# MoFHeka/MeepoEmbedding

Measured on AMD Instinct MI355X. Metric: key-lookups/sec, higher is better.
Workload: dtype int64 keys / fp32 rows (copy)

## Files before the change

include/meepo_embedding.h:

```cpp
#ifndef MEEPO_EMBEDDING_H
#define MEEPO_EMBEDDING_H
#include <stddef.h>
#include <stdint.h>

#ifdef __cplusplus
extern "C" {
#endif

#define MEE_ABI_VERSION 2

#define MEE_EMPTY_KEY     INT64_MIN
#define MEE_RECLAIMED_KEY (INT64_MIN + 1)
#define MEE_BUCKET_WIDTH  16

enum { MEE_OK = 0, MEE_ERR_INVALID_ARG = -1, MEE_ERR_OUT_OF_MEMORY = -2, MEE_ERR_HIP = -3,
       MEE_ERR_NO_DEVICE = -4, MEE_ERR_BATCH_TOO_LARGE = -5, MEE_ERR_UNSUPPORTED = -6,
       MEE_ERR_RCCL = -7  };

enum { MEE_OPT_NONE = 0, MEE_OPT_ADAGRAD = 1, MEE_OPT_ADAM = 2 };
enum { MEE_INIT_CONSTANT = 0, MEE_INIT_UNIFORM = 1 };
enum { MEE_STATUS_TABLE_FULL = 1u, MEE_STATUS_RESERVED_KEY = 2u, MEE_STATUS_STALE_HANDLE = 4u, MEE_STATUS_INTERNAL = 8u };
enum { MEE_MEM_HBM = 0, MEE_MEM_HOST_PINNED = 1 };
enum { MEE_FLAG_TRACK_HITS = 1u, MEE_FLAG_ADMISSION = 2u };

// ... 40 lines not shown
    uint32_t from_env;
    uint32_t placement_consistent;
    float    odd_over_even[2];
    float    block_us_by_index_mod_8[8];
    uint32_t xcc_of_index_mod_8[8];
} mee_calibration;
int mee_device_calibration(int32_t device, mee_calibration* out);

int mee_find(const mee_table* t, const int64_t* d_keys, size_t n, float* d_out, uint8_t* d_found, void* stream);
enum { MEE_FIND_DEFAULT = 0u, MEE_FIND_STREAM_STORES = 1u, MEE_FIND_CACHED_STORES = 2u, MEE_FIND_STREAM_ROWS = 4u, MEE_FIND_STREAM_BUCKETS = 8u };
int mee_find_ex(const mee_table* t, const int64_t* d_keys, size_t n, float* d_out, uint8_t* d_found, uint32_t flags, void* stream);
int mee_find_unordered(const mee_table* t, const int64_t* d_keys, size_t n, float* d_out, uint8_t* d_found, void* stream);
typedef struct mee_find_request { const int64_t* d_keys; size_t n; float* d_out; uint8_t* d_found; } mee_find_request;
int mee_find_many(const mee_table* t, const mee_find_request* reqs, uint32_t count, void* stream);
int mee_find_located(const mee_table* t, const int64_t* d_keys, size_t n, float* d_out, uint8_t* d_found, int64_t* d_slots_out, void* stream);
int mee_find_located_prepare(mee_table* t, const int64_t* d_keys, size_t n, float* d_out, uint8_t* d_found, int64_t* d_slots_out, void* stream);
int mee_find_or_insert_located_prepare(mee_table* t, const int64_t* d_keys, size_t n, float* d_out, uint8_t* d_found, int64_t* d_slots_out, void* stream);
int mee_find_missing(const mee_table* t, const int64_t* d_keys, size_t n, float* d_out, uint8_t* d_found, void* stream);
int mee_find_counted(const mee_table* t, const int64_t* d_keys, size_t n, float* d_out, uint8_t* d_found, int missing_only,
                     void* stream);
int mee_hits_scan(mee_table* t, uint32_t min_hits, uint32_t max_hits, int reset, int64_t* d_keys_out, size_t cap, size_t* n_out,
                  void* stream);
enum { MEE_POOL_SUM = 0, MEE_POOL_MEAN = 1 };
int mee_find_pooled(const mee_table* t, const int64_t* d_keys, size_t n, const uint64_t* d_bag_offsets, size_t n_bags, float* d_out,
                    uint8_t* d_found, int mode, void* stream);
int mee_find_pooled_weighted(const mee_table* t, const int64_t* d_keys, size_t n, const uint64_t* d_bag_offsets, size_t n_bags,
                             const float* d_weights, float* d_out, uint8_t* d_found, int64_t* d_located_out, void* stream);
int mee_pooled_weighted_backward(const mee_table* t, const int64_t* d_keys, const int64_t* d_located, size_t n, const uint64_t* d_bag_offsets,
                                 size_t n_bags, const float* d_weights, const float* d_bag_grads, float* d_grads_out, float* d_weight_grads_out,
                                 void* stream);
enum { MEE_TIER_COUNT_COLD = 1, MEE_TIER_COUNT_HOT = 2 };
int mee_find_pooled_tiered(const mee_table* hot, const mee_table* cold, const int64_t* d_keys, size_t n, const uint64_t* d_bag_offsets, size_t n_bags,
                           void* d_out, uint32_t out_dtype, uint8_t* d_found , int mode, uint32_t flags, void* stream);
int mee_insert(mee_table* t, const int64_t* d_keys, const float* d_values, size_t n, void* stream);
int mee_assign(mee_table* t, const int64_t* d_keys, const float* d_values, size_t n, uint8_t* d_found, void* stream);
int mee_find_plane(const mee_table* t, uint32_t plane, const int64_t* d_keys, size_t n, float* d_out, uint8_t* d_found,
                   void* stream);
int mee_assign_plane(mee_table* t, uint32_t plane, const int64_t* d_keys, const float* d_values, size_t n, uint8_t* d_found,
                     void* stream);
int mee_remove(mee_table* t, const int64_t* d_keys, size_t n, uint8_t* d_found, void* stream);
int mee_find_or_insert(mee_table* t, const int64_t* d_keys, size_t n, float* d_out, uint8_t* d_found, void* stream);
int mee_find_or_insert_located(mee_table* t, const int64_t* d_keys, size_t n, float* d_out, uint8_t* d_found, int64_t* d_slots_out, void* stream);
int mee_find_or_insert_admit(mee_table* t, const int64_t* d_keys, size_t n, float* d_out, uint8_t* d_found, uint32_t min_count, void* stream);
int mee_admission_decay(mee_table* t, uint32_t shift, void* stream);
int mee_insert_missing(mee_table* t, const int64_t* d_keys, const float* d_values, size_t n, const uint8_t* d_found, void* stream);
int mee_find_or_insert_missing(mee_table* t, const int64_t* d_keys, size_t n, float* d_out, const uint8_t* d_found, void* stream);
int mee_export(const mee_table* t, int64_t* d_keys_out, float* d_values_out, float* d_state1_out,
               float* d_state2_out, size_t cap, size_t* n_out, void* stream);
int mee_export_range(const mee_table* t, uint64_t slot_begin, uint64_t slot_end, int64_t* d_keys_out, float* d_values_out,
                     float* d_state1_out, float* d_state2_out, size_t cap, size_t* n_out, void* stream);
int mee_reserve(mee_table* t, uint64_t new_capacity, void* stream);
int mee_size(const mee_table* t, size_t* n_out, void* stream);
int mee_status(const mee_table* t, uint32_t* bits_out, void* stream);
int mee_clear_status(mee_table* t, void* stream);
int mee_locate(const mee_table* t, const int64_t* d_keys, size_t n, int64_t* d_slots_out, uint8_t* d_found, void* stream);
int mee_table_plane(const mee_table* t, uint32_t plane, void** ptr_out, uint64_t* row_stride_bytes, uint32_t* value_memory);
int mee_probe_length(const mee_table* t, const int64_t* d_keys, size_t n, uint64_t* buckets_visited_out, void* stream);
int mee_probe_histogram(const mee_table* t, const int64_t* d_keys, size_t n, uint64_t* hist_out , void* stream);

typedef struct mee_group mee_group;
int mee_group_create(mee_table* const* tables, uint32_t n_tables, uint64_t max_apply_batch, mee_group** out);
int mee_group_destroy(mee_group* g);
int mee_group_set_tuning(mee_group* g, const char* name, int value);
int mee_find_grouped(mee_group* g, const int64_t* d_keys, const uint64_t* d_offsets, size_t n, float* d_out, uint8_t* d_found,
                     void* stream);
int mee_group_find_or_insert(mee_group* g, const int64_t* d_keys, const uint64_t* d_offsets, size_t n, float* d_out, uint8_t* d_found,
// ... 165 lines not shown
```

meepoembedding_amd/_lib.py:

```python
from __future__ import annotations

import ctypes as C
import os

import torch

_HERE = os.path.dirname(os.path.abspath(__file__))
LIB_PATH = os.environ.get("MEE_LIB_PATH") or os.path.join(_HERE, "libmeepo_hip.so")

OK = 0
ERR_INVALID_ARG, ERR_OUT_OF_MEMORY, ERR_HIP, ERR_NO_DEVICE, ERR_BATCH_TOO_LARGE, ERR_UNSUPPORTED, ERR_RCCL = -1, -2, -3, -4, -5, -6, -7
OPT_NONE, OPT_ADAGRAD, OPT_ADAM = 0, 1, 2
INIT_CONSTANT, INIT_UNIFORM = 0, 1
STATUS_TABLE_FULL, STATUS_RESERVED_KEY, STATUS_STALE_HANDLE, STATUS_INTERNAL = 1, 2, 4, 8
FIND_DEFAULT, FIND_STREAM_STORES, FIND_CACHED_STORES, FIND_STREAM_ROWS, FIND_STREAM_BUCKETS = 0, 1, 2, 4, 8
HANDLE_SLOT_MASK = (1 << 40) - 1
MEM_HBM, MEM_HOST_PINNED = 0, 1
DTYPE_F32, DTYPE_BF16 = 0, 1
FLAG_TRACK_HITS, FLAG_ADMISSION = 1, 2
TIER_COUNT_COLD, TIER_COUNT_HOT = 1, 2
ABI_VERSION = 2
EMPTY_KEY = -(1 << 63)
RECLAIMED_KEY = EMPTY_KEY + 1
BUCKET_WIDTH = 16
# ... 65 lines not shown
    "mee_hits_scan": (C.c_int, [_vp, _u32, _u32, C.c_int, _vp, _sz, C.POINTER(_sz), _vp]),
    "mee_insert": (C.c_int, [_vp, _vp, _vp, _sz, _vp]),
    "mee_insert_missing": (C.c_int, [_vp, _vp, _vp, _sz, _vp, _vp]),
    "mee_find_or_insert_missing": (C.c_int, [_vp, _vp, _sz, _vp, _vp, _vp]),
    "mee_assign": (C.c_int, [_vp, _vp, _vp, _sz, _vp, _vp]),
    "mee_find_plane": (C.c_int, [_vp, _u32, _vp, _sz, _vp, _vp, _vp]),
    "mee_assign_plane": (C.c_int, [_vp, _u32, _vp, _vp, _sz, _vp, _vp]),
    "mee_remove": (C.c_int, [_vp, _vp, _sz, _vp, _vp]),
    "mee_find_or_insert": (C.c_int, [_vp, _vp, _sz, _vp, _vp, _vp]),
    "mee_export": (C.c_int, [_vp, _vp, _vp, _vp, _vp, _sz, C.POINTER(_sz), _vp]),
    "mee_group_create": (C.c_int, [C.POINTER(_vp), _u32, _u64, C.POINTER(_vp)]),
    "mee_group_find_pooled": (C.c_int, [_vp, _vp, _sz, _vp, _sz, _vp, _vp, _vp, C.c_int, _vp]),
    "mee_group_apply_adagrad_pooled": (C.c_int, [_vp, _vp, _vp, _sz, _vp, _vp, _vp, _sz, _f32, _f32, _vp]),
    "mee_group_apply_adam_pooled": (C.c_int, [_vp, _vp, _vp, _sz, _vp, _vp, _vp, _sz, _f32, _f32, _f32, _f32, _u64, _vp]),
    "mee_group_find_pooled_jagged": (C.c_int, [_vp, _vp, _sz, _vp, _sz, _vp, _vp, _vp, _vp, C.c_int, _vp]),
    "mee_group_apply_adagrad_indexed": (C.c_int, [_vp, _vp, _vp, _vp, _sz, _vp, _sz, _f32, _f32, _vp]),
    "mee_group_apply_adam_indexed": (C.c_int, [_vp, _vp, _vp, _vp, _sz, _vp, _sz, _f32, _f32, _f32, _f32, _u64, _vp]),
    "mee_group_find_or_insert": (C.c_int, [_vp, _vp, _vp, _sz, _vp, _vp, _vp]),
    "mee_group_apply_adagrad": (C.c_int, [_vp, _vp, _vp, _vp, _sz, _f32, _f32, _vp]),
    "mee_group_apply_adam": (C.c_int, [_vp, _vp, _vp, _vp, _sz, _f32, _f32, _f32, _f32, _u64, _vp]),
    "mee_group_destroy": (C.c_int, [_vp]),
    "mee_group_set_tuning": (C.c_int, [_vp, C.c_char_p, C.c_int]),
    "mee_find_grouped": (C.c_int, [_vp, _vp, _vp, _sz, _vp, _vp, _vp]),
    "mee_mixed_group_create": (C.c_int, [C.POINTER(_vp), _u32, _u64, C.POINTER(_vp)]),
    "mee_mixed_group_destroy": (C.c_int, [_vp]),
    "mee_mixed_group_layout": (C.c_int, [_vp, _u64, C.POINTER(_u64), C.POINTER(_u64)]),
    "mee_mixed_group_find_pooled": (C.c_int, [_vp, _vp, _sz, _vp, _sz, _vp, _u32, _vp, _vp, C.c_int, C.c_int, _vp]),
    "mee_mixed_group_apply_adagrad_pooled": (C.c_int, [_vp, _vp, _vp, _sz, _vp, _vp, _vp, _sz, _f32, _f32, _vp]),
    "mee_mixed_group_apply_adam_pooled": (C.c_int, [_vp, _vp, _vp, _sz, _vp, _vp, _vp, _sz, _f32, _f32, _f32, _f32, _u64, _vp]),
    "mee_mixed_group_set_tuning": (C.c_int, [_vp, C.c_char_p, C.c_int]),
    "mee_find_pooled": (C.c_int, [_vp, _vp, _sz, _vp, _sz, _vp, _vp, C.c_int, _vp]),
    "mee_find_pooled_weighted": (C.c_int, [_vp, _vp, _sz, _vp, _sz, _vp, _vp, _vp, _vp, _vp]),
    "mee_find_pooled_tiered": (C.c_int, [_vp, _vp, _vp, _sz, _vp, _sz, _vp, _u32, _vp, C.c_int, _u32, _vp]),
    "mee_pooled_weighted_backward": (C.c_int, [_vp, _vp, _vp, _sz, _vp, _sz, _vp, _vp, _vp, _vp, _vp]),
    "mee_group_find_pooled_weighted": (C.c_int, [_vp, _vp, _sz, _vp, _sz, _vp, _vp, _vp, _vp, _vp]),
    "mee_group_pooled_weighted_backward": (C.c_int, [_vp, _vp, _vp, _sz, _vp, _sz, _vp, _vp, _vp, _vp, _vp]),
    "mee_apply_adagrad_indexed": (C.c_int, [_vp, _vp, _vp, _sz, _vp, _sz, _f32, _f32, _vp]),
    "mee_apply_adam_indexed": (C.c_int, [_vp, _vp, _vp, _sz, _vp, _sz, _f32, _f32, _f32, _f32, _u64, _vp]),
    "mee_dedup_keys": (C.c_int, [_vp, _vp, _sz, _vp, _vp, C.c_int64, _vp]),
    "mee_reserve": (C.c_int, [_vp, _u64, _vp]),
    "mee_export_range": (C.c_int, [_vp, _u64, _u64, _vp, _vp, _vp, _vp, _sz, C.POINTER(_sz), _vp]),
    "mee_size": (C.c_int, [_vp, C.POINTER(_sz), _vp]),
    "mee_status": (C.c_int, [_vp, C.POINTER(_u32), _vp]),
    "mee_clear_status": (C.c_int, [_vp, _vp]),
    "mee_find_unordered": (C.c_int, [_vp, _vp, _sz, _vp, _vp, _vp]),
    "mee_find_many": (C.c_int, [_vp, C.POINTER(FindRequest), _u32, _vp]),
    "mee_find_located": (C.c_int, [_vp, _vp, _sz, _vp, _vp, _vp, _vp]),
    "mee_find_or_insert_located": (C.c_int, [_vp, _vp, _sz, _vp, _vp, _vp, _vp]),
    "mee_find_located_prepare": (C.c_int, [_vp, _vp, _sz, _vp, _vp, _vp, _vp]),
    "mee_find_or_insert_located_prepare": (C.c_int, [_vp, _vp, _sz, _vp, _vp, _vp, _vp]),
    "mee_apply_adagrad_located": (C.c_int, [_vp, _vp, _vp, _vp, _sz, _f32, _f32, _vp]),
    "mee_apply_adam_located": (C.c_int, [_vp, _vp, _vp, _vp, _sz, _f32, _f32, _f32, _f32, _u64, _vp]),
    "mee_find_or_insert_admit": (C.c_int, [_vp, _vp, _sz, _vp, _vp, _u32, _vp]),
    "mee_admission_decay": (C.c_int, [_vp, _u32, _vp]),
    "mee_locate": (C.c_int, [_vp, _vp, _sz, _vp, _vp, _vp]),
    "mee_table_plane": (C.c_int, [_vp, _u32, C.POINTER(_vp), C.POINTER(_u64), C.POINTER(_u32)]),
    "mee_device_calibration": (C.c_int, [C.c_int32, C.POINTER(Calibration)]),
    "mee_probe_length": (C.c_int, [_vp, _vp, _sz, C.POINTER(_u64), _vp]),
    "mee_probe_histogram": (C.c_int, [_vp, _vp, _sz, C.POINTER(C.c_uint64), _vp]),
    "mee_apply_adagrad": (C.c_int, [_vp, _vp, _vp, _sz, _f32, _f32, _vp]),
    "mee_apply_adam": (C.c_int, [_vp, _vp, _vp, _sz, _f32, _f32, _f32, _f32, _u64, _vp]),
    "mee_apply_prepare": (C.c_int, [_vp, _vp, _sz, _vp]),
    "mee_apply_discard": (C.c_int, [_vp, _vp]),
    "mee_dedup_sum": (C.c_int, [_vp, _vp, _vp, _sz, _vp, _vp, _vp, _vp, C.c_int64, _vp]),
    "mee_hash_batch": (C.c_int, [_vp, _sz, _u64, _u32, _vp, _vp, _vp, _vp]),
    "mee_router_create": (C.c_int, [_i32, _u64, _u32, C.POINTER(_vp)]),
# ... 80 lines not shown
```

meepoembedding_amd/csrc/meepo_find.hip:

```cpp
#include <hip/hip_runtime.h>
#include <hip/hip_ext.h>

#include <cmath>
#include <cstdlib>
#include <cstring>

#include "meepo_apply_part.h"


namespace mee {


template <int DIM4, int R, int NT>
__device__ __forceinline__ void find_span(const int64_t* __restrict__ tkeys, const f32x4* __restrict__ values, uint64_t nb,
                                          const int64_t* __restrict__ keys, uint64_t n, f32x4* __restrict__ out,
                                          uint8_t* __restrict__ found, float defv, uint32_t dim4_rt, uint32_t* hits,
                                          int64_t* __restrict__ slots_out, uint64_t wave, uint64_t n_waves, int64_t handle_tag = 0) {
    const int lane = threadIdx.x & 63, tile = lane >> 4, tl = lane & 15;
    const uint32_t dim4 = DIM4 ? DIM4 : dim4_rt;
    constexpr int KPW = 4 * R;
    const f32x4 def4 = {defv, defv, defv, defv};

    for (uint64_t base = wave * KPW; base < n; base += n_waves * KPW) {
        int64_t key[R];
// ... 148 lines not shown
                           (uint64_t)(m.first_block[q + 1] - m.first_block[q]) * (blockDim.x >> 6));
}

template <int FLAGS>
__global__ __launch_bounds__(256) void find_missing_kernel(const int64_t* __restrict__ tkeys, const float4* __restrict__ values,
                                                           uint64_t nb, uint32_t dim4, const int64_t* __restrict__ keys, uint64_t n,
                                                           float4* __restrict__ out, uint8_t* __restrict__ found, uint32_t* hits) {
    const int lane = threadIdx.x & 63, tile = lane >> 4, tl = lane & 15;
    const uint64_t wave = (uint64_t)blockIdx.x * (blockDim.x >> 6) + (threadIdx.x >> 6);
    const uint64_t n_waves = (uint64_t)gridDim.x * (blockDim.x >> 6);
    for (uint64_t base = wave * 64; base < n; base += n_waves * 64) {
        const uint64_t i = base + lane;
        const int64_t k = i < n ? keys[i] : kEmpty;
        uint64_t rest = __ballot(i < n && found[i] == 0 && !reserved_key(k));
        while (rest) {
            uint64_t mm = rest;
            int p = -1;
            for (int q = 0; q <= tile; ++q) {
                if (mm) { p = __ffsll((unsigned long long)mm) - 1; mm &= mm - 1; } else p = -1;
            }
            const int64_t key = __shfl(k, p >= 0 ? p : 0);
            bool is_new, full;
            const int64_t slot = tile_locate<false, false>(const_cast<int64_t*>(tkeys), nb, key, p >= 0, tile, tl, is_new, full);
            if (p >= 0 && slot >= 0) {
                const uint64_t dst = (base + (uint64_t)p) * dim4, src = (uint64_t)slot * dim4;
                for (uint32_t c = tl; c < dim4; c += 16) out[dst + c] = values[src + c];
                if (tl == 0) {
                    if (FLAGS & 1) found[base + p] = 1;
                    if (FLAGS & 2) atomicAdd(&hits[slot], 1u);
                }
            }
#pragma unroll
            for (int q = 0; q < 4; ++q) rest &= rest - 1;
        }
    }
}

__device__ __forceinline__ bool jagged_member(const uint64_t* __restrict__ member_bags, uint32_t n_members, uint64_t bag, uint64_t& member) {
    uint32_t lo = 0, hi = n_members;
    while (lo < hi) {
        const uint32_t mid = (lo + hi) >> 1;
        if (member_bags[mid + 1] <= bag) lo = mid + 1; else hi = mid;
    }
    member = lo < n_members ? lo : (n_members ? n_members - 1 : 0);
    return lo < n_members && bag >= member_bags[0];
}

template <int DIM4, int U, int BPW, bool GROUPED = false, bool WEIGHTED = false, bool BF16 = false, bool JAGGED = false, bool TIERED = false>
__global__ __launch_bounds__(256) void find_pooled_kernel(const int64_t* __restrict__ tkeys_, const float4* __restrict__ values_,
                                                          uint64_t nb_, const int64_t* __restrict__ keys,
                                                          const uint64_t* __restrict__ offsets, uint64_t n_bags,
                                                          float4* __restrict__ out, uint8_t* __restrict__ found, float defv,
                                                          uint32_t dim4_rt, int mean, const GroupDesc* __restrict__ desc = nullptr,
                                                          uint64_t bags_per_table = 1, int64_t* __restrict__ located = nullptr,
                                                          uint64_t n_keys = ~0ull, const float* __restrict__ weights = nullptr,
                                                          int64_t handle_tag = 0, const uint64_t* __restrict__ member_bags = nullptr,
                                                          uint32_t n_members = 0, TierArgs tier = {}) {
    static_assert(!JAGGED || (GROUPED && !WEIGHTED && !BF16), "the jagged map is the group's plain fp32 lookup");
    static_assert(!TIERED || (!GROUPED && !WEIGHTED && !JAGGED), "the tiered form is one pair's plain sum / mean");
    const int lane = threadIdx.x & 63, tile = lane >> 4, tl = lane & 15;
    const uint64_t wave = (uint64_t)blockIdx.x * (blockDim.x >> 6) + (threadIdx.x >> 6);
    const uint64_t n_waves = (uint64_t)gridDim.x * (blockDim.x >> 6);
    const uint32_t dim4 = DIM4 ? DIM4 : dim4_rt;
    constexpr int C = DIM4 ? DIM4 / 16 : 16;
    constexpr bool TAGGED = WEIGHTED && !GROUPED;
    for (uint64_t b0 = wave * BPW; b0 < n_bags; b0 += n_waves * BPW) {
// ... 518 lines not shown
    if (mode != MEE_POOL_SUM && mode != MEE_POOL_MEAN) return fail(MEE_ERR_INVALID_ARG, "mee_find_pooled_as: mode must be MEE_POOL_SUM or MEE_POOL_MEAN");
    if (d_weights && mode != MEE_POOL_SUM) return fail(MEE_ERR_INVALID_ARG, "mee_find_pooled_as: weighted pooling is MEE_POOL_SUM only");
    if (d_located_out && !d_weights) return fail(MEE_ERR_INVALID_ARG, "mee_find_pooled_as: d_located_out is the weighted form's output (pass weights of 1.0f for a plain sum)");
    return find_pooled_common(t, d_keys, n, d_bag_offsets, n_bags, d_weights, d_out, out_dtype, d_found, d_located_out, mode, stream);
}

int mee_find_pooled_tiered(const mee_table* hot, const mee_table* cold, const int64_t* d_keys, size_t n, const uint64_t* d_bag_offsets, size_t n_bags,
                           void* d_out, uint32_t out_dtype, uint8_t* d_found, int mode, uint32_t flags, void* stream) {
    MEE_RANGE("mee_find_pooled_tiered");
    if (!hot || !cold || (n_bags && (!d_bag_offsets || !d_out)) || (n && !d_keys)) return fail(MEE_ERR_INVALID_ARG, "mee_find_pooled_tiered: null argument");
    if (hot == cold) return fail(MEE_ERR_INVALID_ARG, "mee_find_pooled_tiered: hot and cold are the same table (a key lives in exactly one tier)");
    if (hot->device != cold->device || hot->dim != cold->dim)
        return fail(MEE_ERR_INVALID_ARG, "mee_find_pooled_tiered: the tiers differ in device (%d, %d) or dim (%u, %u)", hot->device, cold->device, hot->dim, cold->dim);
    if (flags & ~(uint32_t)(MEE_TIER_COUNT_COLD | MEE_TIER_COUNT_HOT)) return fail(MEE_ERR_INVALID_ARG, "mee_find_pooled_tiered: unknown flag bits 0x%x", flags);
    if (((flags & MEE_TIER_COUNT_COLD) && !cold->hits) || ((flags & MEE_TIER_COUNT_HOT) && !hot->hits))
        return fail(MEE_ERR_INVALID_ARG, "mee_find_pooled_tiered: a count flag needs that tier created with MEE_FLAG_TRACK_HITS");
    if (int rc = check_out_dtype(d_out, out_dtype, "mee_find_pooled_tiered")) return rc;
    if (mode != MEE_POOL_SUM && mode != MEE_POOL_MEAN) return fail(MEE_ERR_INVALID_ARG, "mee_find_pooled_tiered: mode must be MEE_POOL_SUM or MEE_POOL_MEAN");
    if (n_bags == 0) return MEE_OK;
    DeviceGuard g(hot->device);
    hipStream_t st = as_stream(stream);
    const TierArgs tier{cold->keys, (const float4*)cold->values, cold->nb, (flags & MEE_TIER_COUNT_HOT) ? hot->hits : nullptr,
                        (flags & MEE_TIER_COUNT_COLD) ? cold->hits : nullptr};
    with_pooled_shape(hot->dim4, n, n_bags, [&](auto d4, auto u, auto bpw, unsigned grid) { with_flag(out_dtype == MEE_DTYPE_BF16, [&](auto bf16) {
        constexpr int ut = (bpw == 1 && u > 2) ? 2 : u;
        find_pooled_kernel<d4, ut, bpw, false, false, bf16, false, true><<<grid, 256, 0, st>>>(
            hot->keys, (const float4*)hot->values, hot->nb, d_keys, d_bag_offsets, n_bags, (float4*)d_out, d_found, hot->default_value, hot->dim4,
            mode == MEE_POOL_MEAN, nullptr, 1, nullptr, n, nullptr, 0, nullptr, 0, tier);
    }); });
    MEE_HIP(hipGetLastError());
    return MEE_OK;
}

int mee_pooled_weighted_backward(const mee_table* t, const int64_t* d_keys, const int64_t* d_located, size_t n, const uint64_t* d_bag_offsets,
                                 size_t n_bags, const float* d_weights, const float* d_bag_grads, float* d_grads_out, float* d_weight_grads_out,
                                 void* stream) {
    MEE_RANGE("mee_pooled_weighted_backward");
    if (!t || (n_bags && (!d_bag_offsets || !d_bag_grads)) || (n && (!d_keys || !d_weights || !d_grads_out)))
        return fail(MEE_ERR_INVALID_ARG, "mee_pooled_weighted_backward: null argument");
    if (n_bags == 0) return MEE_OK;
    DeviceGuard g(t->device);
    hipStream_t st = as_stream(stream);
    with_pooled_shape(t->dim4, n, n_bags, [&](auto d4, auto u, auto bpw, unsigned grid) {
        pooled_weighted_backward_kernel<d4, u, bpw><<<grid, 256, 0, st>>>(t->keys, (const float4*)t->values, t->nb, t->capacity, d_keys, d_located, handle_tag_of(t), d_bag_offsets,
                                                                          n_bags, d_weights, (const float4*)d_bag_grads, (float4*)d_grads_out, d_weight_grads_out, t->default_value, t->dim4, nullptr, 1, n);
    });
    MEE_HIP(hipGetLastError());
    return MEE_OK;
}

int mee_find_plane(const mee_table* t, uint32_t plane, const int64_t* d_keys, size_t n, float* d_out, uint8_t* d_found, void* stream) {
    MEE_RANGE("mee_find_plane");
    if (!t || (n && (!d_keys || !d_out))) return fail(MEE_ERR_INVALID_ARG, "mee_find_plane: null argument");
    const float* p = plane_of(t, plane);
    if (!p) return fail(MEE_ERR_UNSUPPORTED, "mee_find_plane: plane %u does not exist (optimizer=%u)", plane, t->optimizer);
    return find_plane(t, p, plane == 0 ? t->default_value : 0.0f, d_keys, n, d_out, d_found, stream);
}

static int group_find_pooled_common(mee_group* g, const int64_t* d_keys, size_t n, const uint64_t* d_bag_offsets, size_t bags_per_table, const float* d_weights,
                                    void* d_out, uint32_t out_dtype, uint8_t* d_found, int64_t* d_located_out, int mode, void* stream) {
    if (bags_per_table == 0) return MEE_OK;
    if (int rc = group_refresh(g, stream)) return rc;
    DeviceGuard guard(g->device);
    hipStream_t st = as_stream(stream);
    const uint64_t n_bags = (uint64_t)g->n_tables * bags_per_table;
    with_pooled_shape(g->dim4, n, n_bags, [&](auto d4, auto u, auto bpw, unsigned grid) { with_flag(d_weights != nullptr, [&](auto weighted) { with_flag(out_dtype == MEE_DTYPE_BF16, [&](auto bf16) {
// ... 116 lines not shown
```

meepoembedding_amd/csrc/meepo_host.h:

```cpp
#pragma once
#include <hip/hip_runtime.h>
#include <cstdarg>
#include <cstdio>
#include <type_traits>

#include "../../include/meepo_embedding.h"

namespace mee {

char* last_error_buf();

inline int fail(int code, const char* fmt, ...) {
    va_list ap;
    va_start(ap, fmt);
    vsnprintf(last_error_buf(), 512, fmt, ap);
    va_end(ap);
    return code;
}

#define MEE_HIP(expr)                                                                                     \
    do {                                                                                                  \
        hipError_t e_ = (expr);                                                                           \
        if (e_ != hipSuccess)                                                                             \
            return ::mee::fail(e_ == hipErrorOutOfMemory ? MEE_ERR_OUT_OF_MEMORY : MEE_ERR_HIP,           \
// ... 20 lines not shown
};
#define MEE_RANGE(name) ::mee::OpRange mee_range_(name)

struct DeviceGuard {
    int prev = -1;
    bool switched = false;
    hipError_t err = hipSuccess;
    explicit DeviceGuard(int device) {
        err = hipGetDevice(&prev);
        if (err == hipSuccess && prev != device) { err = hipSetDevice(device); switched = (err == hipSuccess); }
    }
    ~DeviceGuard() { if (switched) (void)hipSetDevice(prev); }
};

struct TableView {
    int device;
    const int64_t* keys;
    const float* values;
    uint64_t nb;
    uint32_t dim, dim4;
    float default_value;
    uint64_t generation;
    float *s1, *s2;
    uint32_t optimizer;
    uint32_t initializer;
    float init_scale, init_acc;
    uint64_t init_seed;
    uint32_t* status;
    uint32_t* hits;
};
TableView table_view(const mee_table* t);
int find_skip_padding(const mee_table* t, const int64_t* d_keys, size_t n, void* d_out, uint8_t* d_found, void* stream, uint32_t out_dtype = MEE_DTYPE_F32);

struct GroupDesc {
    const int64_t* tkeys;
    float4* values;
    float4* s1;
    float4* s2;
    uint64_t nb;
    float defv;
    uint32_t pad;
};
struct GroupInit {
    uint64_t init_seed;
    uint32_t* status;
    uint32_t* hits;
    uint32_t initializer, optimizer;
    float init_scale, init_acc;
};
constexpr int kGroupSlotBits = 48;
constexpr uint32_t kMaxGroupTables = 1024;

inline unsigned grid_for(size_t work_items, unsigned per_block, unsigned cap) {
    size_t g = (work_items + per_block - 1) / per_block;
    if (g < 1) g = 1;
    if (g > cap) g = cap;
    return (unsigned)g;
}

constexpr uint64_t kCachedOutputBytes = 128ull << 20;

template <class F> decltype(auto) with_row_shape(uint32_t dim4, F&& f) {
    if (dim4 == 16) return f(std::integral_constant<int, 16>{});
    if (dim4 == 32) return f(std::integral_constant<int, 32>{});
    return f(std::integral_constant<int, 0>{});
}
// ... 32 lines not shown
```

meepoembedding_amd/csrc/meepo_sharded.hip:

```cpp
#include <hip/hip_runtime.h>
#include <rccl/rccl.h>

#include <dlfcn.h>

#include <atomic>
#include <cmath>
#include <cstdlib>
#include <cstring>
#include <mutex>
#include <new>
#include <mutex>
#include <unordered_set>
#include <vector>

#include "meepo_device.h"
#include "meepo_host.h"

namespace mee {

struct RcclApi {
    void* handle = nullptr;
    ncclResult_t (*GetUniqueId)(ncclUniqueId*) = nullptr;
    ncclResult_t (*CommInitRank)(ncclComm_t*, int, ncclUniqueId, int) = nullptr;
    ncclResult_t (*CommDestroy)(ncclComm_t) = nullptr;
// ... 373 lines not shown
    Leg legs[2];
    int nl = 0;
    legs[nl++] = Leg{ks, c->recv_keys, 1, 8, ncclInt64};
    if (d_rows) {
        if (int rc = pack_rows(c, d_rows, st)) return rc;
        legs[nl++] = Leg{c->send_rows, c->recv_rows, c->dim, 4, ncclFloat};
    }
    return exchange(c, legs, nl, false, st);
}

static int hot_has_room(mee_sharded* c, uint64_t n, void* stream, bool* room) {
    if (c->hot_ub + n > c->hot_limit) {
        size_t sz = 0;
        if (int rc = mee_size(c->local, &sz, stream)) return rc;
        c->hot_ub = sz;
    }
    *room = c->hot_ub + n <= c->hot_limit;
    return MEE_OK;
}

static int owner_lookup(mee_sharded* c, uint64_t rt, bool insert_missing, void* stream, bool bf16 = false) {
    if (rt == 0) return MEE_OK;
    if (!c->cold && insert_missing) {
        for (uint64_t s = 0; s < rt; s += c->local_max_batch) {
            const uint64_t m = rt - s < c->local_max_batch ? rt - s : c->local_max_batch;
            if (int rc = bf16 ? mee_find_or_insert_as(c->local, c->recv_keys + s, m, (uint16_t*)c->recv_rows + s * c->dim, MEE_DTYPE_BF16, c->recv_found + s, stream)
                              : mee_find_or_insert(c->local, c->recv_keys + s, m, c->recv_rows + s * c->dim, c->recv_found + s, stream)) return rc;
        }
        return MEE_OK;
    }
    if (bf16 && !c->cold)
        return c->cap ? find_skip_padding(c->local, c->recv_keys, rt, c->recv_rows, c->recv_found, stream, MEE_DTYPE_BF16)
                      : mee_find_as(c->local, c->recv_keys, rt, c->recv_rows, MEE_DTYPE_BF16, c->recv_found, MEE_FIND_DEFAULT, stream);
    if (int rc = c->cap ? find_skip_padding(c->local, c->recv_keys, rt, c->recv_rows, c->recv_found, stream)
                        : mee_find(c->local, c->recv_keys, rt, c->recv_rows, c->recv_found, stream)) return rc;
    if (!c->cold) return MEE_OK;
    if (int rc = mee_find_missing(c->cold, c->recv_keys, rt, c->recv_rows, c->recv_found, stream)) return rc;
    for (uint64_t s = 0; insert_missing && s < rt; s += c->local_max_batch) {
        const uint64_t m = rt - s < c->local_max_batch ? rt - s : c->local_max_batch;
        bool room = false;
        if (int rc = hot_has_room(c, m, stream, &room)) return rc;
        if (int rc = mee_find_or_insert_missing(room ? c->local : c->cold, c->recv_keys + s, m, c->recv_rows + s * c->dim, c->recv_found + s, stream)) return rc;
        if (room) c->hot_ub += m;
    }
    if (bf16) {
        shard_narrow_rows_kernel<<<grid_for(rt, 16, 1u << 16), 256, 0, (hipStream_t)stream>>>((const float4*)c->recv_rows, rt, c->dim4, (u32x2*)c->wire_rows);
        MEE_HIP(hipGetLastError());
    }
    return MEE_OK;
}

static int owner_insert(mee_sharded* c, uint64_t rt, void* stream) {
    for (uint64_t s = 0; s < rt; s += c->local_max_batch) {
        const uint64_t m = rt - s < c->local_max_batch ? rt - s : c->local_max_batch;
        const int64_t* k = c->recv_keys + s;
        const float* v = c->recv_rows + s * c->dim;
        if (!c->cold) { if (int rc = mee_insert(c->local, k, v, m, stream)) return rc; continue; }
        if (int rc = mee_assign(c->local, k, v, m, c->recv_found + s, stream)) return rc;
        if (int rc = mee_assign(c->cold, k, v, m, c->recv_found2 + s, stream)) return rc;
        shard_or_kernel<<<grid_for(m, 256, 2048), 256, 0, (hipStream_t)stream>>>(c->recv_found + s, c->recv_found2 + s, m);
        bool room = false;
        if (int rc = hot_has_room(c, m, stream, &room)) return rc;
        if (int rc = mee_insert_missing(room ? c->local : c->cold, k, v, m, c->recv_found + s, stream)) return rc;
        if (room) c->hot_ub += m;
    }
    return MEE_OK;
}

static int owner_assign_or_remove(mee_sharded* c, uint64_t rt, bool assign, void* stream) {
    for (uint64_t s = 0; s < rt; s += c->local_max_batch) {
// ... 396 lines not shown
```

meepoembedding_amd/tiered.py:

```python
from __future__ import annotations

import torch


def _pool_rows(rows: torch.Tensor, bag_offsets: torch.Tensor, mode: str) -> torch.Tensor:
    n = rows.shape[0]
    off = bag_offsets.to(torch.int64)
    end = off[1:].clamp(0, n)
    begin = torch.minimum(off[:-1].clamp(min=0), end)
    lens = end - begin
    out = torch.zeros((lens.numel(), rows.shape[1]), dtype=torch.float32, device=rows.device)
    for j in range(int(lens.max()) if lens.numel() else 0):
        m = lens > j
        r = rows[begin[m] + j]
        out[m] = r if j == 0 else out[m] + r
    if mode == "mean":
        nz = lens > 0
        out[nz] = out[nz] / lens[nz].to(torch.float32)[:, None]
    return out


class TieredLookupTable:
    weighted_bags = False

    def __init__(self, hot, cold, hot_key_limit: int | None = None, sample_every: int = 8, promote_threshold: int = 2,
                 rebalance_every: int = 0, rebalance_max_moves: int = 1 << 20):
        if hot.dim != cold.dim:
            raise ValueError("hot and cold tables must have the same dim")
        self.hot, self.cold, self.dim = hot, cold, hot.dim
        self.supports_pooled_out_dtype = True
        self.optimizer = getattr(hot, "optimizer", 0)
        self.hot_key_limit = int(hot_key_limit if hot_key_limit is not None else getattr(hot, "capacity", 0) * 0.75)
        self._hot_keys_ub = 0
        self.policy = bool(getattr(hot, "track_hits", False) and getattr(cold, "track_hits", False))
        self.sample_every, self.promote_threshold = max(1, sample_every), promote_threshold
        self._calls = 0
        self.rebalance_every, self.rebalance_max_moves = max(0, int(rebalance_every)), int(rebalance_max_moves)
        self._train_steps = 0
        self.rebalance_log: list[tuple[int, int, int]] = []

    @staticmethod
    def _idx(mask: torch.Tensor) -> torch.Tensor:
        return torch.nonzero(mask, as_tuple=False).view(-1)

    def _room_for(self, n_new: int) -> bool:
        if self._hot_keys_ub + n_new > self.hot_key_limit:
            self._hot_keys_ub = self.hot.size()
        return self._hot_keys_ub + n_new <= self.hot_key_limit

    def find(self, keys: torch.Tensor):
        keys = keys.contiguous().view(-1)
        if not self.policy:
            out, found = self.hot.find(keys)
            self.cold.find_missing(keys, out, found)
            return out, found
        self._calls += 1
        if self._calls % self.sample_every == 0:
            out, found = self.hot.find_counted(keys)
        else:
            out, found = self.hot.find(keys)
        self.cold.find_counted(keys, out, found, missing_only=True)
        return out, found

    def _native(self) -> bool:
        from .table import LookupTable
        return isinstance(self.hot, LookupTable) and isinstance(self.cold, LookupTable)

    def find_pooled(self, keys: torch.Tensor, bag_offsets: torch.Tensor, mode: str = "sum", out: torch.Tensor | None = None,
                    found: torch.Tensor | None = None, insert_missing: bool = False, out_dtype: torch.dtype = torch.float32):
        if mode not in ("sum", "mean"):
            raise ValueError(f"mode must be 'sum' or 'mean' (got {mode!r})")
        if not self._native():
            if out_dtype not in (torch.float32, torch.bfloat16):
                raise ValueError(f"out_dtype must be torch.float32 or torch.bfloat16 (got {out_dtype})")
            flat = keys.contiguous().view(-1)
            rows, fnd = self.find_or_insert(flat) if insert_missing else self.find(flat)
            pooled = _pool_rows(rows, bag_offsets, mode).to(out_dtype)
            if out is not None:
                out.copy_(pooled)
            if found is not None:
                found.copy_(fnd)
            return (out if out is not None else pooled), (found if found is not None else fnd)
        from . import _lib
        from .table import _n_bags, _out_dtype
# ... 200 lines not shown
```

Before: 7.899 billion.

## Fuse hot and cold tier lookups into a single tiered find kernel

Result: no change. 7.895 billion (median of 3 runs) (-0.1%).

```diff
diff --git a/include/meepo_embedding.h b/include/meepo_embedding.h
--- a/include/meepo_embedding.h
+++ b/include/meepo_embedding.h
@@ -96,6 +96,8 @@
 enum { MEE_TIER_COUNT_COLD = 1, MEE_TIER_COUNT_HOT = 2 };
 int mee_find_pooled_tiered(const mee_table* hot, const mee_table* cold, const int64_t* d_keys, size_t n, const uint64_t* d_bag_offsets, size_t n_bags,
                            void* d_out, uint32_t out_dtype, uint8_t* d_found , int mode, uint32_t flags, void* stream);
+int mee_find_tiered(const mee_table* hot, const mee_table* cold, const int64_t* d_keys, size_t n, void* d_out, uint32_t out_dtype,
+                    uint8_t* d_found , uint32_t flags, void* stream);
 int mee_insert(mee_table* t, const int64_t* d_keys, const float* d_values, size_t n, void* stream);
 int mee_assign(mee_table* t, const int64_t* d_keys, const float* d_values, size_t n, uint8_t* d_found, void* stream);
 int mee_find_plane(const mee_table* t, uint32_t plane, const int64_t* d_keys, size_t n, float* d_out, uint8_t* d_found,
diff --git a/meepoembedding_amd/_lib.py b/meepoembedding_amd/_lib.py
--- a/meepoembedding_amd/_lib.py
+++ b/meepoembedding_amd/_lib.py
@@ -121,6 +121,7 @@
     "mee_find_pooled": (C.c_int, [_vp, _vp, _sz, _vp, _sz, _vp, _vp, C.c_int, _vp]),
     "mee_find_pooled_weighted": (C.c_int, [_vp, _vp, _sz, _vp, _sz, _vp, _vp, _vp, _vp, _vp]),
     "mee_find_pooled_tiered": (C.c_int, [_vp, _vp, _vp, _sz, _vp, _sz, _vp, _u32, _vp, C.c_int, _u32, _vp]),
+    "mee_find_tiered": (C.c_int, [_vp, _vp, _vp, _sz, _vp, _u32, _vp, _u32, _vp]),
     "mee_pooled_weighted_backward": (C.c_int, [_vp, _vp, _vp, _sz, _vp, _sz, _vp, _vp, _vp, _vp, _vp]),
     "mee_group_find_pooled_weighted": (C.c_int, [_vp, _vp, _sz, _vp, _sz, _vp, _vp, _vp, _vp, _vp]),
     "mee_group_pooled_weighted_backward": (C.c_int, [_vp, _vp, _vp, _sz, _vp, _sz, _vp, _vp, _vp, _vp, _vp]),
diff --git a/meepoembedding_amd/csrc/meepo_find.hip b/meepoembedding_amd/csrc/meepo_find.hip
--- a/meepoembedding_amd/csrc/meepo_find.hip
+++ b/meepoembedding_amd/csrc/meepo_find.hip
@@ -204,6 +204,159 @@
             }
 #pragma unroll
             for (int q = 0; q < 4; ++q) rest &= rest - 1;
+        }
+    }
+}
+
+template <int NT>
+__device__ __forceinline__ void store_row4(f32x4* __restrict__ out, uint64_t idx, const f32x4& v) {
+    if constexpr ((NT & 256) != 0) store_bf16x4<(NT & 4) != 0>(out, idx, v);
+    else { if (NT & 4) out[idx] = v; else __builtin_nontemporal_store(v, &out[idx]); }
+}
+
+template <int DIM4, int R, int NT>
+__global__ __launch_bounds__(256) void find_tiered_kernel(const int64_t* __restrict__ tkeys, const f32x4* __restrict__ values, uint64_t nb, const TierArgs cold,
+                                                          const int64_t* __restrict__ keys, uint64_t n, f32x4* __restrict__ out, uint8_t* __restrict__ found,
+                                                          float defv, uint32_t dim4_rt) {
+    const int lane = threadIdx.x & 63, tile = lane >> 4, tl = lane & 15;
+    const uint64_t wave = (uint64_t)blockIdx.x * (blockDim.x >> 6) + (threadIdx.x >> 6), n_waves = (uint64_t)gridDim.x * (blockDim.x >> 6);
+    const uint32_t dim4 = DIM4 ? DIM4 : dim4_rt;
+    constexpr int KPW = 4 * R;
+    const f32x4 def4 = {defv, defv, defv, defv};
+    const f32x4* __restrict__ cvalues = reinterpret_cast<const f32x4*>(cold.values);
+
+    for (uint64_t base = wave * KPW; base < n; base += n_waves * KPW) {
+        int64_t key[R], slot[R], kb[R];
+        uint64_t b[R];
+        bool inb[R], act[R], hit[R];
+        const int64_t kmine = (lane < KPW && base + lane < n) ? keys[base + lane] : kEmpty;
+#pragma unroll
+        for (int r = 0; r < R; ++r) {
+            const uint64_t i = base + r * 4 + tile;
+            inb[r] = i < n;
+            key[r] = __shfl(kmine, r * 4 + tile);
+            act[r] = inb[r] && !reserved_key(key[r]);
+            if constexpr ((NT & 128) != 0) {
+                if (inb[r] && !act[r] && tl == 0 && found) found[i] = 1;
+                inb[r] = act[r];
+            }
+        }
+#pragma unroll
+        for (int r = 0; r < R; ++r) {
+            b[r] = bucket_of(key[r], nb);
+            kb[r] = act[r] ? tkeys[b[r] * kW + tl] : kEmpty;
+        }
+#pragma unroll
+        for (int r = 0; r < R; ++r) slot[r] = tile_probe(tkeys, nb, key[r], act[r], b[r], kb[r], tile, tl);
+        bool missed = false;
+#pragma unroll
+        for (int r = 0; r < R; ++r) { hit[r] = slot[r] >= 0; missed = missed || (act[r] && !hit[r]); }
+        if (!__any(missed)) {
+            if constexpr (DIM4 != 0) {
+                constexpr int C = DIM4 / 16;
+                f32x4 row[R][C];
+                bool all_hit = true;
+#pragma unroll
+                for (int r = 0; r < R; ++r) all_hit = all_hit && inb[r] && slot[r] >= 0;
+                if (__all(all_hit)) {
+#pragma unroll
+                    for (int r = 0; r < R; ++r)
+#pragma unroll
+                        for (int c = 0; c < C; ++c) row[r][c] = values[(uint64_t)slot[r] * DIM4 + c * 16 + tl];
+#pragma unroll
+                    for (int r = 0; r < R; ++r)
+#pragma unroll
+                        for (int c = 0; c < C; ++c) store_row4<NT>(out, (base + r * 4 + tile) * DIM4 + c * 16 + tl, row[r][c]);
+                } else {
+#pragma unroll
+                    for (int r = 0; r < R; ++r)
+#pragma unroll
+                        for (int c = 0; c < C; ++c) row[r][c] = slot[r] >= 0 ? values[(uint64_t)slot[r] * DIM4 + c * 16 + tl] : def4;
+#pragma unroll
+                    for (int r = 0; r < R; ++r)
+                        if (inb[r]) {
+#pragma unroll
+                            for (int c = 0; c < C; ++c) store_row4<NT>(out, (base + r * 4 + tile) * DIM4 + c * 16 + tl, row[r][c]);
+                        }
+                }
+            } else {
+#pragma unroll
+                for (int r = 0; r < R; ++r)
+                    if (inb[r])
+                        for (uint32_t c = tl; c < dim4; c += 16)
+                            store_row4<NT>(out, (base + r * 4 + tile) * dim4 + c, slot[r] >= 0 ? values[(uint64_t)slot[r] * dim4 + c] : def4);
+            }
+        } else {
+            int64_t cslot[R];
+            bool cact[R];
+            if constexpr (DIM4 != 0) {
+                constexpr int C = DIM4 / 16;
+                f32x4 row[R][C];
+#pragma unroll
+                for (int r = 0; r < R; ++r) {
+                    cact[r] = act[r] && !hit[r];
+                    b[r] = bucket_of(key[r], cold.nb);
+                    kb[r] = cact[r] ? cold.tkeys[b[r] * kW + tl] : kEmpty;
+                }
+#pragma unroll
+                for (int r = 0; r < R; ++r) cslot[r] = tile_probe(cold.tkeys, cold.nb, key[r], cact[r], b[r], kb[r], tile, tl);
+#pragma unroll
+                for (int r = 0; r < R; ++r) {
+                    const f32x4* src = hit[r] ? values + (uint64_t)slot[r] * DIM4 : cslot[r] >= 0 ? cvalues + (uint64_t)cslot[r] * DIM4 : values;
+#pragma unroll
+                    for (int c = 0; c < C; ++c) row[r][c] = src[c * 16 + tl];
+                }
+#pragma unroll
+                for (int r = 0; r < R; ++r)
+#pragma unroll
+                    for (int c = 0; c < C; ++c) row[r][c] = (hit[r] || cslot[r] >= 0) ? row[r][c] : def4;
+#pragma unroll
+                for (int r = 0; r < R; ++r)
+                    if (inb[r]) {
+#pragma unroll
+                        for (int c = 0; c < C; ++c) store_row4<NT>(out, (base + r * 4 + tile) * DIM4 + c * 16 + tl, row[r][c]);
+                    }
+            } else {
+#pragma unroll
+                for (int r = 0; r < R; ++r) {
+                    cact[r] = act[r] && !hit[r];
+                    b[r] = bucket_of(key[r], cold.nb);
+                    kb[r] = cact[r] ? cold.tkeys[b[r] * kW + tl] : kEmpty;
+                }
+#pragma unroll
+                for (int r = 0; r < R; ++r) cslot[r] = tile_probe(cold.tkeys, cold.nb, key[r], cact[r], b[r], kb[r], tile, tl);
+#pragma unroll
+                for (int r = 0; r < R; ++r) {
+                    const f32x4* src = slot[r] >= 0 ? values + (uint64_t)slot[r] * dim4 : cvalues + (uint64_t)(cslot[r] >= 0 ? cslot[r] : 0) * dim4;
+                    const bool any = slot[r] >= 0 || cslot[r] >= 0;
+                    if (inb[r])
+                        for (uint32_t c = tl; c < dim4; c += 16) store_row4<NT>(out, (base + r * 4 + tile) * dim4 + c, any ? src[c] : def4);
+                }
+            }
+#pragma unroll
+            for (int r = 0; r < R; ++r) hit[r] = hit[r] || cslot[r] >= 0;
+            if (cold.cold_hits) {
+#pragma unroll
+                for (int r = 0; r < R; ++r)
+                    if (cslot[r] >= 0 && tl == 0) atomicAdd(&cold.cold_hits[cslot[r]], 1u);
+            }
+        }
+        if (cold.hot_hits) {
+#pragma unroll
+            for (int r = 0; r < R; ++r)
+                if (slot[r] >= 0 && tl == 0) atomicAdd(&cold.hot_hits[slot[r]], 1u);
+        }
+        if (found) {
+#pragma unroll
+            for (int r = 0; r < R; ++r) {
+                const uint64_t i0 = base + r * 4;
+                if ((NT & 128) == 0 && i0 + 4 <= n && (reinterpret_cast<uintptr_t>(found) & 3) == 0) {
+                    const uint64_t m = __ballot(hit[r]);
+                    const uint32_t w = (uint32_t)(m & 1) | ((uint32_t)((m >> 16) & 1) << 8) | ((uint32_t)((m >> 32) & 1) << 16) |
+                                       ((uint32_t)((m >> 48) & 1) << 24);
+                    if (lane == 0) *reinterpret_cast<uint32_t*>(found + i0) = w;
+                } else if (inb[r] && tl == 0) found[i0 + tile] = hit[r];
+            }
         }
     }
 }
@@ -788,6 +941,49 @@
     return MEE_OK;
 }
 
+}
+namespace mee {
+int find_tiered(const mee_table* hot, const mee_table* cold, const int64_t* d_keys, size_t n, void* d_out, uint32_t out_dtype, uint8_t* d_found, uint32_t flags,
+                void* stream, bool skip_padding, const char* name) {
+    if (!hot || !cold || (n && (!d_keys || !d_out || (skip_padding && !d_found)))) return fail(MEE_ERR_INVALID_ARG, "%s: null argument", name);
+    if (hot == cold) return fail(MEE_ERR_INVALID_ARG, "%s: hot and cold are the same table (a key lives in exactly one tier)", name);
+    if (hot->device != cold->device || hot->dim != cold->dim)
+        return fail(MEE_ERR_INVALID_ARG, "%s: the tiers differ in device (%d, %d) or dim (%u, %u)", name, hot->device, cold->device, hot->dim, cold->dim);
+    if (flags & ~(uint32_t)(MEE_TIER_COUNT_COLD | MEE_TIER_COUNT_HOT)) return fail(MEE_ERR_INVALID_ARG, "%s: unknown flag bits 0x%x", name, flags);
+    if (((flags & MEE_TIER_COUNT_COLD) && !cold->hits) || ((flags & MEE_TIER_COUNT_HOT) && !hot->hits))
+        return fail(MEE_ERR_INVALID_ARG, "%s: a count flag needs that tier created with MEE_FLAG_TRACK_HITS", name);
+    if (int rc = check_out_dtype(d_out, out_dtype, name)) return rc;
+    const bool bf16 = out_dtype == MEE_DTYPE_BF16;
+    if (skip_padding && bf16) return fail(MEE_ERR_UNSUPPORTED, "%s: the padded form writes fp32 rows", name);
+    if (n == 0) return MEE_OK;
+    DeviceGuard g(hot->device);
+    hipStream_t st = as_stream(stream);
+    const uint64_t out_bytes = (uint64_t)n * hot->dim * (bf16 ? 2 : 4);
+    const bool cached_out = hot->find_nt >= 0 ? (hot->find_nt & 4) != 0 : (out_bytes <= kCachedOutputBytes && !outputs_rotate(hot, d_out, out_bytes));
+    const TierArgs tier{cold->keys, (const float4*)cold->values, cold->nb, (flags & MEE_TIER_COUNT_HOT) ? hot->hits : nullptr,
+                        (flags & MEE_TIER_COUNT_COLD) ? cold->hits : nullptr};
+    with_row_shape(hot->dim4, [&](auto d4) {
+        constexpr int D4 = d4;
+        constexpr int R = RowShape<D4>::rows_per_tile;
+        const unsigned grid = grid_for(n, 4u * 4u * (unsigned)R, 1u << 22);
+        auto launch = [&](auto ntc) {
+            find_tiered_kernel<D4, R, ntc><<<grid, 256, 0, st>>>(hot->keys, (const f32x4*)hot->values, hot->nb, tier, d_keys, n, (f32x4*)d_out, d_found, hot->default_value, hot->dim4);
+        };
+        const int nt = (cached_out ? 4 : 0) | (skip_padding ? 128 : 0) | (bf16 ? 256 : 0);
+        with_value<0, 4, 128, 132, 256, 260>(nt, launch);
+    });
+    MEE_HIP(hipGetLastError());
+    return MEE_OK;
+}
+}
+extern "C" {
+
+int mee_find_tiered(const mee_table* hot, const mee_table* cold, const int64_t* d_keys, size_t n, void* d_out, uint32_t out_dtype, uint8_t* d_found, uint32_t flags,
+                    void* stream) {
+    MEE_RANGE("mee_find_tiered");
+    return find_tiered(hot, cold, d_keys, n, d_out, out_dtype, d_found, flags, stream, false, "mee_find_tiered");
+}
+
 int mee_pooled_weighted_backward(const mee_table* t, const int64_t* d_keys, const int64_t* d_located, size_t n, const uint64_t* d_bag_offsets,
                                  size_t n_bags, const float* d_weights, const float* d_bag_grads, float* d_grads_out, float* d_weight_grads_out,
                                  void* stream) {
diff --git a/meepoembedding_amd/csrc/meepo_host.h b/meepoembedding_amd/csrc/meepo_host.h
--- a/meepoembedding_amd/csrc/meepo_host.h
+++ b/meepoembedding_amd/csrc/meepo_host.h
@@ -76,6 +76,9 @@
 TableView table_view(const mee_table* t);
 int find_skip_padding(const mee_table* t, const int64_t* d_keys, size_t n, void* d_out, uint8_t* d_found, void* stream, uint32_t out_dtype = MEE_DTYPE_F32);
 
+int find_tiered(const mee_table* hot, const mee_table* cold, const int64_t* d_keys, size_t n, void* d_out, uint32_t out_dtype, uint8_t* d_found, uint32_t flags,
+                void* stream, bool skip_padding, const char* name);
+
 struct GroupDesc {
     const int64_t* tkeys;
     float4* values;
diff --git a/meepoembedding_amd/csrc/meepo_sharded.hip b/meepoembedding_amd/csrc/meepo_sharded.hip
--- a/meepoembedding_amd/csrc/meepo_sharded.hip
+++ b/meepoembedding_amd/csrc/meepo_sharded.hip
@@ -429,10 +429,14 @@
     if (bf16 && !c->cold)
         return c->cap ? find_skip_padding(c->local, c->recv_keys, rt, c->recv_rows, c->recv_found, stream, MEE_DTYPE_BF16)
                       : mee_find_as(c->local, c->recv_keys, rt, c->recv_rows, MEE_DTYPE_BF16, c->recv_found, MEE_FIND_DEFAULT, stream);
-    if (int rc = c->cap ? find_skip_padding(c->local, c->recv_keys, rt, c->recv_rows, c->recv_found, stream)
-                        : mee_find(c->local, c->recv_keys, rt, c->recv_rows, c->recv_found, stream)) return rc;
-    if (!c->cold) return MEE_OK;
-    if (int rc = mee_find_missing(c->cold, c->recv_keys, rt, c->recv_rows, c->recv_found, stream)) return rc;
+    if (c->cold && !bf16) {
+        if (int rc = find_tiered(c->local, c->cold, c->recv_keys, rt, c->recv_rows, MEE_DTYPE_F32, c->recv_found, 0, stream, c->cap != 0, "mee_sharded_find")) return rc;
+    } else {
+        if (int rc = c->cap ? find_skip_padding(c->local, c->recv_keys, rt, c->recv_rows, c->recv_found, stream)
+                            : mee_find(c->local, c->recv_keys, rt, c->recv_rows, c->recv_found, stream)) return rc;
+        if (!c->cold) return MEE_OK;
+        if (int rc = mee_find_missing(c->cold, c->recv_keys, rt, c->recv_rows, c->recv_found, stream)) return rc;
+    }
     for (uint64_t s = 0; insert_missing && s < rt; s += c->local_max_batch) {
         const uint64_t m = rt - s < c->local_max_batch ? rt - s : c->local_max_batch;
         bool room = false;
diff --git a/meepoembedding_amd/tiered.py b/meepoembedding_amd/tiered.py
--- a/meepoembedding_amd/tiered.py
+++ b/meepoembedding_amd/tiered.py
@@ -50,6 +50,19 @@
 
     def find(self, keys: torch.Tensor):
         keys = keys.contiguous().view(-1)
+        if self._native():
+            from . import _lib
+            hot, cold = self.hot, self.cold
+            k = hot._keys(keys)
+            n = k.numel()
+            out = torch.empty((n, self.dim), dtype=torch.float32, device=hot.device)
+            found = torch.empty(n, dtype=torch.uint8, device=hot.device)
+            flags = 0
+            if self.policy:
+                self._calls += 1
+                flags = _lib.TIER_COUNT_COLD | (_lib.TIER_COUNT_HOT if self._calls % self.sample_every == 0 else 0)
+            _lib.check(_lib.lib().mee_find_tiered(hot._h, cold._h, k.data_ptr(), n, out.data_ptr(), _lib.DTYPE_F32, found.data_ptr(), flags, hot._s()))
+            return out, found
         if not self.policy:
             out, found = self.hot.find(keys)
             self.cold.find_missing(keys, out, found)
```
